# buq2/camera_calibrator

Hardware: AMD Instinct MI355X
Metric: LM residuals/sec (2*N_obs per LM iteration), single-camera intrinsics BA (higher is better)
Workload: dtype f64; 1 GPU; BASELINE.json configs[2]: single-camera intrinsics, 1000 frames x 500 pts per GPU, radial-tangential distortion, Zhang init, reference solver options (calibrator.cpp:314-321); frames_total=1000, points_per_frame=500, observations_total=500000, parallelism=frame-sharded x1, exchange=none

## Files before the change

camera_calibrator_amd/csrc/cc_intrinsics.hip:

```cpp
#include "cc_common.hpp"
#include "cc_device.hpp"
#include "cc_intrinsics_dev.hpp"
#include "cc_intrinsics_persist.hpp"


#include <algorithm>
#include <chrono>
#include <climits>
#include <cstdlib>
#include <cstring>
#include <vector>

namespace cc {

__global__ __launch_bounds__(kSweepThreads, 4) void k_intr_sweep(IntrDev P, int flags) {
  extern __shared__ __attribute__((aligned(16))) char smem_raw[];
  double* s_stage = reinterpret_cast<double*>(smem_raw);
  double* s_blk = s_stage;
  double* sm = s_stage + 4 * kStageDoublesPerWave;
  const int tid = threadIdx.x, lane = tid & 63, wave = tid >> 6;
  const int T = P.T;
  const int64_t f = (int64_t)blockIdx.x / T;
  const int tile = (int)(blockIdx.x - f * T);
  const bool in_solve = (flags & 1) != 0, restart = (flags & 2) != 0;
// ... 863 lines not shown
}

namespace cc {
int intr_create_impl(cc_intrinsics* h, const int64_t* off, const float* uv, const float* xyz);
static thread_local bool g_create_one_shot = false;
static thread_local bool g_create_no_obs = false;
static thread_local size_t g_create_extra = 0;
struct OneShotCreate {
  OneShotCreate(size_t extra, bool no_obs = false) { g_create_one_shot = true; g_create_extra = extra; g_create_no_obs = no_obs; }
  ~OneShotCreate() { g_create_one_shot = false; g_create_extra = 0; g_create_no_obs = false; }
};
static double ms_since(std::chrono::steady_clock::time_point t0) { return std::chrono::duration<double, std::milli>(std::chrono::steady_clock::now() - t0).count(); }
}

extern "C" {

void cc_intrinsics_destroy(cc_intrinsics* h);

int cc_intrinsics_create(int32_t device, int64_t F, const int64_t* off, const float* uv,
                         const float* xyz, cc_intrinsics** out) {
  using namespace cc;
  if (!out || !off || F <= 0) return fail(CC_ERR_BAD_ARGUMENT, "cc_intrinsics_create: bad arguments");
  if (off[0] != 0) return fail(CC_ERR_BAD_ARGUMENT, "frame_offsets[0] must be 0");
  for (int64_t f = 0; f < F; ++f)
    if (off[f + 1] < off[f]) return fail(CC_ERR_BAD_ARGUMENT, "frame_offsets must be non-decreasing");
  const int64_t N = off[F];
  if (F >= ((int64_t)1 << 28) || N >= ((int64_t)1 << 40))
    return fail(CC_ERR_BAD_ARGUMENT, "cc_intrinsics_create: problem too large (frames < 2^28, observations < 2^40)");
  if (N > 0 && (!uv || !xyz) && !cc::g_create_no_obs) return fail(CC_ERR_BAD_ARGUMENT, "uv/xyz are NULL");
  if (int rc = select_device(device)) return rc;
  cc_intrinsics* h = new cc_intrinsics();
  h->device = device; h->F = F; h->N = N;
  h->one_shot = cc::g_create_one_shot;
  h->no_obs_upload = cc::g_create_no_obs;
  h->extra_bytes = cc::g_create_extra;
  const int rc_init = cc::intr_create_impl(h, off, uv, xyz);
  if (rc_init != CC_OK) {
    cc_intrinsics_destroy(h);
    return rc_init;
  }
  *out = h;
  return CC_OK;
}

int cc_intrinsics_exchange_export(cc_intrinsics* h, uint8_t handle[64]) {
  using namespace cc;
  if (h && handle && h->huber_a > 0.0) return fail(CC_ERR_STATE, "cc_intrinsics_exchange_export: the handle has a Huber loss set (one device only)");
  if (h && handle && h->model != CC_MODEL_RADTAN) return fail(CC_ERR_STATE, "cc_intrinsics_exchange_export: the handle has the fisheye model set (one device only)");
  if (int rc = exchange_export_begin(h, handle, "cc_intrinsics_exchange_export")) return rc;
  h->d.x = P2pDev{};
  return mailbox_export(&h->mailbox, kVecSolve, 16, handle);
}

int cc_intrinsics_exchange_attach(cc_intrinsics* h, int32_t rank, int32_t nranks, const uint8_t* handles) {
  using namespace cc;
  if (!h || !handles || rank < 0 || nranks < 1 || rank >= nranks || nranks > kP2pMaxRanks)
    return fail(CC_ERR_BAD_ARGUMENT, "cc_intrinsics_exchange_attach: bad arguments (nranks must be 1..%d)", kP2pMaxRanks);
  if (h->huber_a > 0.0) return fail(CC_ERR_STATE, "cc_intrinsics_exchange_attach: the handle has a Huber loss set (one device only)");
  if (h->model != CC_MODEL_RADTAN) return fail(CC_ERR_STATE, "cc_intrinsics_exchange_attach: the handle has the fisheye model set (one device only)");
  if (!h->mailbox.local) return fail(CC_ERR_STATE, "cc_intrinsics_exchange_attach: call cc_intrinsics_exchange_export first");
  if (h->comm) return fail(CC_ERR_STATE, "cc_intrinsics_exchange_attach: an RCCL communicator is already attached");
  CC_HIP(hipSetDevice(h->device));
  drop_graphs(h);
  if (int rc = mailbox_attach(&h->mailbox, rank, nranks, handles, &h->d.x)) return rc;
  h->d.rank = rank;
  h->d.nranks = nranks;
  h->exchange = true;
  h->persist_x_ok = false;
  if (h->persist_ok) {
    int ndev = 1;
    if (hipGetDeviceCount(&ndev) != hipSuccess || ndev < 1) ndev = 1;
    const int co = getenv("CC_INTR_CO_RESIDENT") ? std::max(1, atoi(getenv("CC_INTR_CO_RESIDENT"))) : (nranks + ndev - 1) / ndev;
    h->persist_x_ok = (int64_t)(h->pq.G + 1) * co <= h->p_resident;
  }
  if (nranks > 1) {
    double* d_out = nullptr;
    int* d_ok = nullptr;
    CC_HIP(hipMalloc(&d_out, sizeof(double)));
    CC_HIP(hipMalloc(&d_ok, sizeof(int)));
    hipLaunchKernelGGL(k_intr_flag_exchange, dim3(1), dim3(64), 0, h->stream, h->d, h->persist_x_ok ? 1.0 : 0.0, d_out, d_ok);
    double sum = 0.0;
    int ok = 0;
    const hipError_t e1 = hipMemcpyAsync(&sum, d_out, sizeof(double), hipMemcpyDeviceToHost, h->stream);
    const hipError_t e2 = hipMemcpyAsync(&ok, d_ok, sizeof(int), hipMemcpyDeviceToHost, h->stream);
    const hipError_t e3 = hipStreamSynchronize(h->stream);
    hipFree(d_out);
    hipFree(d_ok);
    CC_HIP(e1); CC_HIP(e2); CC_HIP(e3);
    if (!ok) return fail(CC_ERR_COMM, "cc_intrinsics_exchange_attach: a peer rank did not attach within 10 s");
    h->persist_x_ok = sum == (double)nranks;
  }
  return CC_OK;
}

}

namespace cc {
int intr_create_impl(cc_intrinsics* h, const int64_t* off, const float* uv, const float* xyz) {
  const int64_t F = h->F, N = h->N;
  if (int rc = stream_get(h->device, &h->stream)) return rc;
  IntrDev& d = h->d;
  d.F = F; d.N = N; d.rank = 0; d.nranks = 1; d.mask = 0;
  {
    const int64_t per_frame = F > 0 ? (N + F - 1) / F : 0;
    int64_t T = std::min<int64_t>((per_frame + 2 * kSweepThreads - 1) / (2 * kSweepThreads), 256 / std::max<int64_t>(F, 1));
    if (const char* env = getenv("CC_SWEEP_TILES")) T = atoi(env);
    d.T = (int32_t)std::max<int64_t>(1, std::min<int64_t>(T, 8));
    d.tpad_ = 0;
    if (F * d.T >= (int64_t)INT32_MAX)
      return fail(CC_ERR_BAD_ARGUMENT, "cc_intrinsics_create: %lld frames x %d sweep tiles exceed the launch grid", (long long)F, (int)d.T);
  }
  const size_t FT = (size_t)F * d.T;
  const size_t n1 = (size_t)std::max<int64_t>(N, 1);
  size_t cursor = 0;
  auto take = [&](size_t bytes) { const size_t at = cursor; cursor += (bytes + 255) & ~(size_t)255; return at; };
  d.log_cap = 4096;
  const size_t o_intr = take(2 * 16 * sizeof(double));
  const size_t o_pose = take((size_t)2 * F * 8 * sizeof(double));
  const size_t o_stats = take(FT * kStatsCols * sizeof(double));
  const size_t o_hd0 = take(FT * 16 * sizeof(double));
  const size_t o_sp = take((size_t)F * 8 * sizeof(double));
  const size_t o_Y = take((size_t)F * kYStride * sizeof(double));
  const size_t o_partial = take((size_t)kElimMaxBlocks * kPartialCols * sizeof(double));
  const size_t o_vs = take(kVecSolve * sizeof(double));
  const size_t o_vd = take(16 * sizeof(double));
  const size_t o_ds = take(16 * sizeof(double));
  const size_t o_ss = take(16 * sizeof(double));
  const size_t o_ctl = take(sizeof(LmCtl));
  const size_t o_ctln = take(sizeof(LmCtl));
  const size_t o_sync = take(64);
  const size_t o_opts = take(sizeof(LmOpts));
  const size_t o_iintr = take(16 * sizeof(double));
  const size_t o_ipose = take((size_t)F * 8 * sizeof(double));
  int p_teams = 0;
  const bool want_persist = d.T == 1 && !(getenv("CC_INTR_PERSIST") && atoi(getenv("CC_INTR_PERSIST")) == 0);
  if (want_persist) {
    for (int t = 1; t <= kPMaxTeams && !p_teams; t *= 2) {
      int resident = 0;
      if (int rc = persist_resident_workgroups(h->device, t, &resident)) return rc;
      if ((F + t - 1) / t + 1 <= resident && (F + t - 1) / t <= kPMaxWorkers) { p_teams = t; h->p_resident = resident; }
    }
    if (const char* e = getenv("CC_INTR_PERSIST_TEAMS")) {
      const int t = atoi(e);
      int resident = 0;
      if ((t == 1 || t == 2 || t == 4) && !persist_resident_workgroups(h->device, t, &resident) && (F + t - 1) / t + 1 <= resident && (F + t - 1) / t <= kPMaxWorkers) { p_teams = t; h->p_resident = resident; }
    }
  }
  const int64_t PG = p_teams ? (F + p_teams - 1) / p_teams : 1;
  const size_t pgn = (size_t)PG;
  const size_t o_pbox0 = cursor;
  const size_t o_sbox = take(pgn * 2 * kPStatCols * sizeof(unsigned long long));
  const size_t o_pbox = take(pgn * 2 * kPartialCols * sizeof(unsigned long long));
  const size_t o_rbox = take(pgn * 2 * kPartialCols * sizeof(unsigned long long));
  const size_t o_lbox = take(((pgn + kPLeaderRows - 1) / kPLeaderRows) * 2 * kPartialCols * sizeof(unsigned long long));
  const size_t o_xbox = take(kPBcastWords * sizeof(unsigned long long));
  const size_t o_pfail = take(64);
  h->p_box_bytes = cursor - o_pbox0;
  const size_t zeroed = cursor;
  const size_t o_blocks = take((size_t)2 * FT * 256 * sizeof(double));
  const size_t o_log = take((size_t)d.log_cap * sizeof(cc_iteration));
  const size_t o_uv = take(n1 * 2 * sizeof(float));
  const size_t o_xyz = take(n1 * 3 * sizeof(float));
  const size_t o_off = take((size_t)(F + 1) * sizeof(int64_t));
  const size_t o_extra = take(h->extra_bytes);
  if (int rc = arena_get(h->device, cursor, &h->arena, &h->arena_cached)) return rc;
  char* base = static_cast<char*>(h->arena);
  h->extra = h->extra_bytes ? base + o_extra : nullptr;
  CC_HIP(hipMemsetAsync(base, 0, zeroed, h->stream));
  if (N > 0 && !h->no_obs_upload) {
    CC_HIP(hipMemcpyAsync(base + o_uv, uv, (size_t)N * 2 * sizeof(float), hipMemcpyHostToDevice, h->stream));
    CC_HIP(hipMemcpyAsync(base + o_xyz, xyz, (size_t)N * 3 * sizeof(float), hipMemcpyHostToDevice, h->stream));
  }
  CC_HIP(hipMemcpyAsync(base + o_off, off, (size_t)(F + 1) * sizeof(int64_t), hipMemcpyHostToDevice, h->stream));
  if (!h->one_shot) CC_HIP(hipStreamSynchronize(h->stream));
  d.uv = reinterpret_cast<const float*>(base + o_uv);
  d.xyz = reinterpret_cast<const float*>(base + o_xyz);
  d.off = reinterpret_cast<const int64_t*>(base + o_off);
  d.intr = reinterpret_cast<double*>(base + o_intr);
  d.pose = reinterpret_cast<double*>(base + o_pose);
  d.blocks = reinterpret_cast<double*>(base + o_blocks);
  d.stats = reinterpret_cast<double*>(base + o_stats);
  d.hd0 = reinterpret_cast<double*>(base + o_hd0);
  d.sp = reinterpret_cast<double*>(base + o_sp);
  d.Y = reinterpret_cast<double*>(base + o_Y);
  d.partial = reinterpret_cast<double*>(base + o_partial);
  d.vec_solve = reinterpret_cast<double*>(base + o_vs);
  d.vec_decide = reinterpret_cast<double*>(base + o_vd);
  d.ds = reinterpret_cast<double*>(base + o_ds);
  d.ss = reinterpret_cast<double*>(base + o_ss);
  d.ctl = reinterpret_cast<LmCtl*>(base + o_ctl);
  d.ctl_next = reinterpret_cast<LmCtl*>(base + o_ctln);
  d.arrive = reinterpret_cast<unsigned*>(base + o_sync);
  d.pub_seq = reinterpret_cast<unsigned long long*>(base + o_sync + 8);
  d.opts = reinterpret_cast<LmOpts*>(base + o_opts);
  d.log = reinterpret_cast<cc_iteration*>(base + o_log);
  h->init_intr = reinterpret_cast<double*>(base + o_iintr);
  h->init_pose = reinterpret_cast<double*>(base + o_ipose);
  d.init_intr = h->init_intr;
  d.init_pose = h->init_pose;
  static_assert(16 + sizeof(LmCtl) <= 192 && sizeof(LmCtl) <= 160 && sizeof(LmOpts) <= 160, "one cached 512-byte pinned block holds all three");
  h->pinned = pinned_block_get();
  if (!h->pinned) return fail(CC_ERR_HIP, "hipHostMalloc failed");
  h->host_pub = reinterpret_cast<volatile unsigned long long*>(h->pinned);
  h->h_ctl = reinterpret_cast<LmCtl*>(static_cast<char*>(h->pinned) + 192);
  h->h_opts = reinterpret_cast<LmOpts*>(static_cast<char*>(h->pinned) + 352);
  h->host_pub[0] = 0ull;
  h->pub_count = 0;
  {
    void* dev_view = nullptr;
    CC_HIP(hipHostGetDevicePointer(&dev_view, h->pinned, 0));
    d.host_pub = reinterpret_cast<unsigned long long*>(dev_view);
  }
  h->pq.sbox = reinterpret_cast<unsigned long long*>(base + o_sbox);
  h->pq.pbox = reinterpret_cast<unsigned long long*>(base + o_pbox);
  h->pq.rbox = reinterpret_cast<unsigned long long*>(base + o_rbox);
  h->pq.xbox = reinterpret_cast<unsigned long long*>(base + o_xbox);
  h->pq.fail = reinterpret_cast<unsigned*>(base + o_pfail);
  h->pq.lbox = reinterpret_cast<unsigned long long*>(base + o_lbox);
  h->pq.G = (int32_t)PG;
  h->pq.teams = p_teams;
  h->p_epoch = 0;
  h->persist_ok = p_teams != 0;
  h->elim_blocks = (int)std::min<int64_t>(kElimMaxBlocks, (F + 15) / 16);
  CC_HIP(hipFuncSetAttribute(reinterpret_cast<const void*>(k_intr_sweep),
                             hipFuncAttributeMaxDynamicSharedMemorySize, kSweepLdsBytes));
  CC_HIP(hipFuncSetAttribute(reinterpret_cast<const void*>(k_intr_sweep_huber),
                             hipFuncAttributeMaxDynamicSharedMemorySize, kSweepLdsBytes));
  CC_HIP(hipFuncSetAttribute(reinterpret_cast<const void*>(k_intr_sweep_fisheye),
                             hipFuncAttributeMaxDynamicSharedMemorySize, kSweepLdsBytes));
  return CC_OK;
}
}

extern "C" {

void cc_intrinsics_destroy(cc_intrinsics* h) {
  if (h) cc::last_call_status_record(h->ran_form >= 0 ? h->ran_form : cc_intrinsics_solver_form(h), h->form_reruns, h->form_note);
  if (!h) return;
  hipSetDevice(h->device);
  bool stream_ok = true;
  if (h->stream) {
    hipStreamCaptureStatus cap = hipStreamCaptureStatusNone;
    stream_ok = hipStreamSynchronize(h->stream) == hipSuccess &&
                hipStreamIsCapturing(h->stream, &cap) == hipSuccess && cap == hipStreamCaptureStatusNone;
    (void)hipGetLastError();
  }
  cc::drop_graphs(h);
  for (auto e : h->events) hipEventDestroy(e);
  if (h->comm) cc::comm_destroy(h->comm);
  cc::exchange_release(h);
  if (h->arena) cc::arena_put(h->device, h->arena, h->arena_cached);
  cc::pinned_block_put(h->pinned);
  if (stream_ok) cc::stream_put(h->device, h->stream);
  else if (h->stream) hipStreamDestroy(h->stream);
  delete h;
}

int cc_intrinsics_set_state(cc_intrinsics* h, const double* intr9, uint32_t mask, const double* q,
                            const double* t) {
  using namespace cc;
  if (!h || !intr9 || !q || !t) return fail(CC_ERR_BAD_ARGUMENT, "cc_intrinsics_set_state: NULL argument");
  CC_HIP(hipSetDevice(h->device));
  std::vector<double> pose((size_t)h->F * 8, 0.0);
  for (int64_t f = 0; f < h->F; ++f) {
    for (int i = 0; i < 4; ++i) pose[f * 8 + i] = q[f * 4 + i];
    for (int i = 0; i < 3; ++i) pose[f * 8 + 4 + i] = t[f * 3 + i];
  }
  double k[16] = {0};
  for (int i = 0; i < 9; ++i) k[i] = intr9[i];
  if (h->model == CC_MODEL_FISHEYE) { k[8] = 0.0; mask |= 1u << 8; }
  CC_HIP(hipStreamSynchronize(h->stream));
  CC_HIP(hipMemcpy(h->init_intr, k, sizeof(k), hipMemcpyHostToDevice));
  CC_HIP(hipMemcpy(h->init_pose, pose.data(), pose.size() * sizeof(double), hipMemcpyHostToDevice));
  if (h->d.mask != (mask & 0x1ffu)) drop_graphs(h);
  h->d.mask = mask & 0x1ffu;
  h->have_state = true;
  return cc_intrinsics_reset(h);
}

int cc_intrinsics_reset(cc_intrinsics* h) {
  using namespace cc;
  if (!h || !h->have_state) return fail(CC_ERR_STATE, "cc_intrinsics_reset: no state set");
  h->ctl_fresh = true;
  h->reset_pending = true;
  return CC_OK;
}

int cc_intrinsics_get_state(cc_intrinsics* h, double* intr9, double* q, double* t) {
  using namespace cc;
  if (!h) return fail(CC_ERR_BAD_ARGUMENT, "cc_intrinsics_get_state: NULL handle");
  CC_HIP(hipSetDevice(h->device));
  LmCtl c;
  if (int rc = read_ctl(h, &c)) return rc;
  const int cur = c.cur & 1;
  if (intr9) CC_HIP(hipMemcpy(intr9, h->d.intr + cur * 16, 9 * sizeof(double), hipMemcpyDeviceToHost));
  if (q || t) {
    std::vector<double> pose((size_t)h->F * 8);
    CC_HIP(hipMemcpy(pose.data(), h->d.pose + (size_t)cur * h->F * 8, pose.size() * sizeof(double), hipMemcpyDeviceToHost));
    for (int64_t f = 0; f < h->F; ++f) {
      if (q) for (int i = 0; i < 4; ++i) q[f * 4 + i] = pose[f * 8 + i];
      if (t) for (int i = 0; i < 3; ++i) t[f * 3 + i] = pose[f * 8 + 4 + i];
    }
  }
  return CC_OK;
}

int cc_intrinsics_eval(cc_intrinsics* h, double* blocks, double* cost) {
// ... 726 lines not shown
```

camera_calibrator_amd/csrc/cc_intrinsics_persist.hip:

```cpp
#include "cc_intrinsics_persist.hpp"
#include "cc_persist_dev.hpp"

namespace cc {


constexpr int persist_lds_doubles(int teams) { return teams * 4 * kStageDoublesPerWave + teams * 2 * 256 + teams * 192 + 512; }

enum { TM_Y = 0, TM_POSE = 60, TM_SP = 76, TM_STEP = 84, TM_R = 100, TM_T = 109, TM_KC = 112, TM_STEP2 = 122, TM_XN2 = 123,
       TM_QW = 124, TM_STAT = 128  };
enum { WG_INTR = 0 , WG_X = 64 , WG_DS = 66 ,
       WG_SS = 80 , WG_R0 = 96 , WG_OPT = 100 ,
       WG_TAB = 104 ,
       WG_TGI = 416 , WG_TZ = 456  };

static_assert(TM_POSE - TM_Y >= 6 * 10 && TM_SP - TM_POSE >= 2 * 8 && TM_STEP - TM_SP >= 6 && TM_R - TM_STEP >= 15 && TM_T - TM_R >= 9 && TM_KC - TM_T >= 3 &&
              TM_STEP2 - TM_KC >= 9 && TM_QW - TM_XN2 >= 1 && TM_STAT - TM_QW >= 4 && TM_STAT + 4 + 9 <= 192,
              "per-team scratch: Y (6 x 10), two poses, pose scale, step (9 + 6), R, t, intrinsics, scalars, statistics row -- inside the 192 doubles persist_lds_doubles gives a team");
static_assert(WG_X - WG_INTR >= 2 * 16 && WG_DS - WG_X >= 2 && WG_SS - WG_DS >= 9 && WG_R0 - WG_SS >= 9 && WG_OPT - WG_R0 >= 1 && WG_TAB - WG_OPT >= 4 &&
              WG_TZ - WG_TGI >= 80 / 2 && WG_TZ + 80 / 2 <= 512,
              "workgroup scratch: both intrinsics, broadcast (2 + 9), scales, options, tables of the 80-slot row -- inside the 512 doubles of persist_lds_doubles");

template <int NC, int NG, int BATCH = 8>
__device__ __forceinline__ void gather_rows(const u64* box, int G, unsigned tag, int ncols, int maxcol, double* s_part,
                                            double* out, unsigned* fail, int* s_ok, int tshift) {
  const int tid = threadIdx.x, col = tid % NC, grp = tid / NC;
  if (tid == 0) *s_ok = 1;
  __syncthreads();
  if (grp < NG && col < ncols) {
    double acc = 0.0;
    bool good = true;
    const long long t0 = wall_clock64();
    for (int r0 = grp; r0 < G && good; r0 += BATCH * NG) {
      u64 lo[BATCH], hi[BATCH];
      for (unsigned spins = 0;; ++spins) {
#pragma unroll
        for (int u = 0; u < BATCH; ++u) {
          const int r = r0 + u * NG;
          const u64* p = box + (size_t)(r < G ? r : r0) * (2 * NC) + 2 * col;
          lo[u] = ag_ld(p);
          hi[u] = ag_ld(p + 1);
        }
        bool ok = true;
#pragma unroll
        for (int u = 0; u < BATCH; ++u) ok = ok && (unsigned)(lo[u] >> 32) == tag && (unsigned)(hi[u] >> 32) == tag;
        if (ok) break;
        if ((spins & 63u) == 63u && (timed_out(t0, tshift) || ag_ld32(fail) != 0u)) { good = false; break; }
        __builtin_amdgcn_s_sleep(1);
      }
      if (!good) break;
#pragma unroll
      for (int u = 0; u < BATCH; ++u) {
        if (r0 + u * NG < G) {
          const double v = ungranule(lo[u], hi[u]);
          acc = col == maxcol ? fmax(acc, v) : acc + v;
        }
      }
    }
    s_part[grp * NC + col] = acc;
    if (!good) *s_ok = 0;
  }
  __syncthreads();
  if (tid < ncols) {
    double a = 0.0;
    if (tid == maxcol) { for (int g = 0; g < NG; ++g) a = fmax(a, s_part[g * NC + tid]); }
    else { for (int g = 0; g < NG; ++g) a += s_part[g * NC + tid]; }
    out[tid] = a;
  }
  __syncthreads();
}

template <int THREADS>
__device__ __forceinline__ void gather_stats4(const u64* box, int G, unsigned tag, double* s_part, double* out, unsigned* fail, int* s_ok, int tshift) {
  constexpr int RPT = 1024 / THREADS;
  static_assert(THREADS / 4 * RPT == kPMaxWorkers, "one statistics row per four threads: the host caps the worker grid at kPMaxWorkers");
  const int tid = threadIdx.x, col = tid & 3, lane = tid & 63, wave = tid >> 6;
  if (tid == 0) *s_ok = 1;
  __syncthreads();
  u64 lo[RPT], hi[RPT];
  bool good = true;
  const long long t0 = wall_clock64();
  for (unsigned spins = 0;; ++spins) {
    bool ok = true;
#pragma unroll
    for (int k = 0; k < RPT; ++k) {
      const int r = (tid >> 2) + k * (THREADS / 4);
      const u64* p = box + (size_t)(r < G ? r : 0) * (2 * kPStatCols) + 2 * col;
      lo[k] = ag_ld(p);
      hi[k] = ag_ld(p + 1);
    }
#pragma unroll
    for (int k = 0; k < RPT; ++k) ok = ok && (unsigned)(lo[k] >> 32) == tag && (unsigned)(hi[k] >> 32) == tag;
    if (ok) break;
    if ((spins & 63u) == 63u && (timed_out(t0, tshift) || ag_ld32(fail) != 0u)) { good = false; break; }
    __builtin_amdgcn_s_sleep(1);
  }
  double acc = 0.0;
#pragma unroll
  for (int k = 0; k < RPT; ++k)
    if ((tid >> 2) + k * (THREADS / 4) < G) acc += ungranule(lo[k], hi[k]);
  acc = wave_sum_mod<2>(acc);
  if (lane < 4) s_part[wave * 4 + lane] = acc;
  if (!good) *s_ok = 0;
  __syncthreads();
  if (tid < 4) {
    double a = 0.0;
#pragma unroll
    for (int w = 0; w < THREADS / 64; ++w) a += s_part[w * 4 + tid];
    out[tid] = a;
  }
  __syncthreads();
}

template <int THREADS>
__device__ __forceinline__ void persist_control(const IntrDev& P, const PersistDev& Q, double* lds) {
  double* s_part = lds;
  double* sv = lds + 1024;
  double* s_tot = lds + 1152;
  double* s_bc = lds + 1168;
  double* s_intr = lds + 1184;
  double* s_ss = lds + 1216;
  LmCtl* s_ctl = reinterpret_cast<LmCtl*>(lds + 1232);
  LmOpts* s_opts = reinterpret_cast<LmOpts*>(lds + 1252);
  cc_iteration* s_log = reinterpret_cast<cc_iteration*>(lds + 1264);
  int* s_int = reinterpret_cast<int*>(lds + 1296);
  const int tid = threadIdx.x, wave = tid >> 6;
  static_assert(sizeof(cc_iteration) <= 32 * 8, "log record scratch");
  if (tid < (int)(sizeof(LmCtl) / 8)) reinterpret_cast<double*>(s_ctl)[tid] = 0.0;
  if (tid >= 32 && tid < 32 + (int)(sizeof(LmOpts) / 8)) reinterpret_cast<u64*>(s_opts)[tid - 32] = reinterpret_cast<const u64*>(P.opts)[tid - 32];
  if (tid >= 64 && tid < 64 + 32) s_intr[tid - 64] = 0.0;
  __syncthreads();
  if (tid < 9) s_intr[tid] = (Q.restart ? P.init_intr : P.intr)[tid];
  if (tid == 0) s_int[1] = 0;
  __syncthreads();
  const LmOpts& o = *s_opts;
  const uint32_t mask = P.mask;

  for (int round = 0; round < Q.max_rounds; ++round) {
    const unsigned e1 = Q.epoch0 + 3u * (unsigned)round + 1u, e2 = e1 + 1u, e3 = e1 + 2u;
    const bool phase0 = round == 0;
    if (phase0) gather_rows<kPStatCols, THREADS / kPStatCols>(Q.sbox, Q.G, e1, 13, -1, s_part, s_tot, Q.fail, s_int, (phase0 ? Q.first_shift : Q.timeout_shift));
    else gather_stats4<THREADS>(Q.sbox, Q.G, e1, s_part, s_tot, Q.fail, s_int, (phase0 ? Q.first_shift : Q.timeout_shift));
    if (P.x.on) {
      const bool need = phase0 || (s_ctl->cand_pending && s_ctl->step_valid);
      if (need) {
        if (tid >= 13 && tid < 16) s_tot[tid] = 0.0;
        __syncthreads();
        const unsigned long long epoch = P.x.seq[1] + 1ull;
        p2p_post(P.x, 1, epoch, P.rank, P.nranks, s_tot, 16);
        int* s_ok2 = s_int + 4;
        const double a = p2p_collect(P.x, 1, epoch, P.rank, P.nranks, 16, s_ok2);
        if (tid < 16) s_tot[tid] = a;
        if (tid == 0) { P.x.seq[1] = epoch; if (!*s_ok2) s_int[0] = 0; }
        __syncthreads();
      }
    }
    if (tid == 0) {
      LmCtl c = *s_ctl;
      const int len0 = c.log_len, prev_cur = c.cur & 1, was_valid = c.step_valid;
      const double prev_radius = c.radius;
      const double* kc0 = s_intr + (c.cur ? 16 : 0);
      const double* kc1 = s_intr + (c.cur ? 0 : 16);
      if (!s_int[0]) {
        __hip_atomic_store(Q.fail, 1u, __ATOMIC_RELAXED, __HIP_MEMORY_SCOPE_AGENT);
        c.done = 1; c.term = CC_FAILURE_EXCHANGE;
      } else if (phase0) {
        double xn2 = s_tot[ST_XNORM2];
#pragma unroll
        for (int i = 0; i < 9; ++i) {
          const double ki = kc0[i];
          xn2 += ki * ki;
          s_ss[i] = o.jacobi_scaling ? 1.0 / (1.0 + sqrt(s_tot[4 + i])) : 1.0;
        }
        lm_init(c, o, s_tot[ST_COST], sqrt(xn2));
      } else if (c.cand_pending) {
        double step2 = s_tot[ST_STEP2], xn2 = s_tot[ST_XNORM2];
        if (c.step_valid) {
#pragma unroll
          for (int i = 0; i < 9; ++i) {
            const double kc = kc1[i], k0 = kc0[i];
            const double d = kc - k0;
            step2 += d * d;
            xn2 += kc * kc;
          }
        }
        lm_decide(c, o, s_log, s_tot[ST_COST], s_tot[ST_QMODEL], step2, xn2);
      }
      if (!c.done && round + 1 >= Q.max_rounds) { c.done = 1; c.term = CC_NO_CONVERGENCE; }
      *s_ctl = c;
      s_int[1] = c.log_len != len0;
      s_int[2] = phase0 ? (!c.done && c.radius == o.initial_radius)
                        : (was_valid && !c.done && (c.cur & 1) == (prev_cur ^ 1) && c.radius == persist_spec_radius(prev_radius, o.max_radius));
      s_bc[0] = (double)((c.done ? 1 : 0) | ((c.cur & 1) << 3));
      s_bc[1] = c.radius;
#pragma unroll
      for (int i = 0; i < 9; ++i) s_bc[2 + i] = 0.0;
    }
    __syncthreads();
    const bool hit = s_int[2] != 0;
    if (s_ctl->done || !hit) {
      if (tid < 22) ag_st(Q.xbox + tid, granule(e2, s_bc[tid >> 1], tid & 1));
      if (s_ctl->done) {
        if (tid == 0 && s_int[1] && s_ctl->log_len <= P.log_cap) P.log[s_ctl->log_len - 1] = *s_log;
        break;
      }
    }
    const unsigned erow = hit ? e2 : e3;
    gather_rows<kPartialCols, THREADS / kPartialCols, (kPLeaderRows + THREADS / kPartialCols - 1) / (THREADS / kPartialCols)>(Q.lbox, (Q.G + kPLeaderRows - 1) / kPLeaderRows, erow, kPartialCols, PC_GMAXP, s_part, sv, Q.fail, s_int, (phase0 ? Q.first_shift : Q.timeout_shift));
    if (P.x.on) {
      if (tid >= kPartialCols && tid < kVecSolve) sv[tid] = 0.0;
      __syncthreads();
      if (tid == 0) { sv[kPartialCols + P.rank] = sv[PC_GMAXP]; sv[PC_GMAXP] = 0.0; }
      __syncthreads();
      const unsigned long long epoch = P.x.seq[0] + 1ull;
      p2p_post(P.x, 0, epoch, P.rank, P.nranks, sv, kVecSolve);
      int* s_ok2 = s_int + 4;
      const double a = p2p_collect(P.x, 0, epoch, P.rank, P.nranks, kVecSolve, s_ok2);
      if (tid < kVecSolve) sv[tid] = a;
      if (tid == 0) { P.x.seq[0] = epoch; if (!*s_ok2) s_int[0] = 0; }
      __syncthreads();
      if (tid == 0) {
        double g = 0.0;
        for (int r = 0; r < P.nranks && r < 32; ++r) g = fmax(g, sv[kPartialCols + r]);
        sv[PC_GMAXP] = g;
      }
      __syncthreads();
    }
    if (wave == 0) {
      int lane = tid & 63;
      asm volatile("" : "+v"(lane));
      const int cur = s_ctl->cur & 1;
      const double radius = s_ctl->radius;
      const double gl = (lane < 9 && !((mask >> lane) & 1u)) ? fabs(sv[PC_GS + lane]) : sv[PC_GMAXP];
      const double k_l = s_intr[cur * 16 + (lane < 9 ? lane : 8)], ss_l = s_ss[lane < 9 ? lane : 8];
      bool ok = !(sv[PC_FAIL] > 0.0);
      double x[9];
      {
#pragma clang fp contract(off)
        const int i = lane < 9 ? lane : 8;
        const bool pin_i = (mask >> i) & 1u;
        const double si = s_ss[i];
        const double damp = clampd(sv[PC_HDIAG + i] * (si * si), o.min_lm_diagonal, o.max_lm_diagonal) / radius;
        double a[9];
#pragma unroll
        for (int k = 0; k < 9; ++k) {
          const int kk = k <= i ? k : i;
          const int idx = kk * 9 - kk * (kk - 1) / 2 + (i - kk);
          double v = sv[idx] * (s_ss[kk] * si);
          if (k == i) v += damp;
          const bool pin_k = (mask >> kk) & 1u;
          if (pin_i || pin_k) v = (k == i) ? 1.0 : 0.0;
          a[k] = v;
        }
        const double b = pin_i ? 0.0 : sv[PC_B + i] * si;
        ok = chol_solve_rows<9>(a, b, x) && ok;
#pragma unroll
        for (int j = 0; j < 9; ++j) ok = ok && isfinite(x[j]);
      }
      const double gmax = row16_max(gl);
      const bool go = s_int[0] && !(gmax <= o.gradient_tolerance) && !(radius < o.min_radius);
      if (lane < 9) {
        double xs = 0.0;
#pragma unroll
        for (int j = 0; j < 9; ++j) xs = lane == j ? x[j] : xs;
        const double ds = go ? -xs : 0.0;
        const double d = ((mask >> lane) & 1u) ? 0.0 : ds * ss_l;
        s_bc[2 + lane] = d;
        s_intr[(cur ^ 1) * 16 + lane] = k_l + d;
      }
      if (lane == 0) {
        s_bc[0] = (double)((go ? 0 : 1) | (go && ok ? 2 : 0) | (hit ? 4 : 0) | (cur << 3));
        s_bc[1] = radius;
        s_bc[12] = gmax;
      }
      wave_lds_fence();
      if (lane < 22) ag_st(Q.xbox + lane, granule(erow, s_bc[lane >> 1], lane & 1));
    }
    if (tid == 0) {
      const double gmax = s_bc[12];
      const bool ok = ((int)s_bc[0] & 2) != 0;
      cc_iteration* e = s_int[1] ? s_log : nullptr;
      if (e && e->accepted) e->gradient_max_norm = gmax;
      if (!s_int[0]) { __hip_atomic_store(Q.fail, 1u, __ATOMIC_RELAXED, __HIP_MEMORY_SCOPE_AGENT); s_ctl->done = 1; s_ctl->term = CC_FAILURE_EXCHANGE; }
      else if (lm_finalize(*s_ctl, o, gmax)) { s_ctl->step_valid = ok ? 1 : 0; s_ctl->cand_pending = 1; }
      if (e && s_ctl->log_len <= P.log_cap) P.log[s_ctl->log_len - 1] = *e;
    }
    __syncthreads();
    if (s_ctl->done) break;
  }
  __syncthreads();
  if (tid < 32 && ag_ld32(Q.fail) == 0u) P.intr[tid] = s_intr[tid];
  if (tid == 0) {
    LmCtl c = *s_ctl;
    if (ag_ld32(Q.fail) != 0u) { c.done = 1; c.term = CC_FAILURE_EXCHANGE; }
    if (!c.done) { c.done = 1; c.term = CC_NO_CONVERGENCE; }
    *P.ctl = c;
    *P.ctl_next = c;
    publish_to_host(P, c);
  }
}

template <int TEAMS>
__global__ __launch_bounds__(TEAMS * 256, TEAMS) void k_intr_persist(IntrDev P, PersistDev Q) {
  constexpr int THREADS = TEAMS * 256;
  extern __shared__ __attribute__((aligned(16))) char smem_raw[];
  double* s_stage = reinterpret_cast<double*>(smem_raw);
  if ((int)blockIdx.x == Q.G) { persist_control<THREADS>(P, Q, s_stage); return; }
  double* s_G = s_stage + TEAMS * 4 * kStageDoublesPerWave;
  double* s_tm = s_G + TEAMS * 2 * 256;
  double* s_wg = s_tm + TEAMS * 192;
#define CC_FRESH_TID(name) int name = tid0; asm volatile("" : "+v"(name))
  const int tid0 = threadIdx.x, wave = __builtin_amdgcn_readfirstlane(tid0 >> 6), team = wave >> 2, twave = wave & 3;
  const int sbase = (team & 3) * 64;
  const int64_t f = (int64_t)blockIdx.x * TEAMS + team;
  const bool has_frame = f < P.F;
  double* sm = s_tm + team * 192;
  double* tstage = s_stage + team * 4 * kStageDoublesPerWave;
  double* s_blk = tstage;
  double* Zs = tstage + 1024;
  double* red = tstage + 1100;
  unsigned char* pj = reinterpret_cast<unsigned char*>(s_wg + WG_TAB);
  unsigned char* pk = pj + 48;
  const uint32_t mask = P.mask;

  {
  const int tid = tid0, ttid = tid0 & 255;
  if (has_frame && ttid < 8) {
    const double v = ttid < 7 ? (Q.restart ? P.init_pose : P.pose)[(size_t)f * 8 + ttid] : 0.0;
    sm[TM_POSE + ttid] = v;
    sm[TM_POSE + 8 + ttid] = v;
  }
  if (ttid >= 64 && ttid < 64 + 60) sm[TM_Y + ttid - 64] = 0.0;
  if (tid < 32) s_wg[WG_INTR + tid] = 0.0;
  if (tid == 32) {
    const LmOpts* o = P.opts;
    s_wg[WG_OPT] = o->jacobi_scaling ? 1.0 : 0.0;
    s_wg[WG_OPT + 1] = o->min_lm_diagonal;
    s_wg[WG_OPT + 2] = o->max_lm_diagonal;
    s_wg[WG_OPT + 3] = o->max_radius;
    s_wg[WG_R0] = o->initial_radius;
  }
  if (tid == 33) {
    int oo = 0;
    for (int j = 0; j < 9; ++j)
      for (int k = j; k < 9; ++k) { pj[oo] = (unsigned char)j; pk[oo] = (unsigned char)k; ++oo; }
  }
  if (tid >= 64 && tid < 64 + 16) s_wg[WG_X + tid - 64] = 0.0;
  if (tid >= 80 && tid < 80 + 16) s_wg[WG_SS + tid - 80] = 1.0;
  __syncthreads();
  if (tid < 9) s_wg[WG_INTR + tid] = (Q.restart ? P.init_intr : P.intr)[tid];
  if (tid >= 128 && tid < 128 + kPartialCols) {
    const int o = tid - 128;
    int gi = 0, z = 0;
    if (o < 45) {
      const int j = pj[o], k = pk[o];
      gi = j * 16 + k; z = j | (k << 8) | (1 << 16);
    } else if (o < 54) {
      const int j = o - 45;
      gi = j * 16 + 15; z = j | (9 << 8) | (1 << 16);
    } else if (o < 63) {
      const int j = o - 54;
// ... 146 lines not shown
        sm[TM_STAT + ST_QMODEL] = (sm[TM_QW] + sm[TM_QW + 1]) + (sm[TM_QW + 2] + sm[TM_QW + 3]);
        sm[TM_STAT + ST_STEP2] = sm[TM_STEP2];
        sm[TM_STAT + ST_XNORM2] = sm[TM_XN2];
      }
      if (phase0 && ttid < 9 * 17 && ttid % 17 == 0) sm[TM_STAT + 4 + ttid / 17] = g;
      __syncthreads();
    }
    {
      CC_FRESH_TID(tid);
      const int ncols = phase0 ? 13 : 4;
      const int stid = tid - 128;
      if (stid >= 0 && stid < 2 * ncols) {
        const int c = stid >> 1;
        double a = 0.0;
        if (do_sweep) {
#pragma unroll
          for (int k = 0; k < TEAMS; ++k)
            if ((int64_t)blockIdx.x * TEAMS + k < P.F) a += s_tm[k * 192 + TM_STAT + c];
        }
        ag_st(Q.sbox + (size_t)blockIdx.x * (2 * kPStatCols) + stid, granule(e1, a, stid & 1));
      }
    }
    auto eliminate_and_post = [&](const int cur_e, const double radius_e, const bool first, u64* box, const unsigned tag) {
    CC_FRESH_TID(tid_e);
    if (has_frame && (tid_e & 255) >= sbase && (tid_e & 255) < sbase + 16) {
      const int l = (tid_e & 255) - sbase;
      const double* Gl = s_G + (team * 2 + cur_e) * 256;
      const double* ss = s_wg + WG_SS;
      const bool jac = s_wg[WG_OPT] != 0.0;
      const double mn = s_wg[WG_OPT + 1], mx = s_wg[WG_OPT + 2];
      const double inv_radius = 1.0 / radius_e;
      double s[6], L[21];
#pragma unroll
      for (int i = 0; i < 6; ++i)
#pragma unroll
        for (int j = 0; j <= i; ++j) L[tri(i, j)] = Gl[(9 + i) * 16 + 9 + j];
      if (first) {
#pragma unroll
        for (int i = 0; i < 6; ++i) s[i] = jac ? 1.0 / (1.0 + sqrt(L[tri(i, i)])) : 1.0;
        if (l < 6) {
          double sl = 0.0;
#pragma unroll
          for (int i = 0; i < 6; ++i) sl = l == i ? s[i] : sl;
          sm[TM_SP + l] = sl;
        }
      } else {
#pragma unroll
        for (int i = 0; i < 6; ++i) s[i] = sm[TM_SP + i];
      }
#pragma unroll
      for (int i = 0; i < 6; ++i)
#pragma unroll
        for (int j = 0; j <= i; ++j) L[tri(i, j)] = s[i] * L[tri(i, j)] * s[j];
#pragma unroll
      for (int i = 0; i < 6; ++i) L[tri(i, i)] += clampd(L[tri(i, i)], mn, mx) * inv_radius;
      bool ok = true;
      double Li[6];
#pragma unroll
      for (int j = 0; j < 6; ++j) {
        double d = L[tri(j, j)];
#pragma unroll
        for (int k = 0; k < j; ++k) d -= L[tri(j, k)] * L[tri(j, k)];
        ok = ok && (d > 0.0) && isfinite(d);
        const double inv = rsqrt_pos(d);
        L[tri(j, j)] = d * inv;
        Li[j] = inv;
#pragma unroll
        for (int i = j + 1; i < 6; ++i) {
          double a = L[tri(i, j)];
#pragma unroll
          for (int k = 0; k < j; ++k) a -= L[tri(i, k)] * L[tri(j, k)];
          L[tri(i, j)] = a * inv;
        }
      }
#pragma unroll
      for (int i = 0; i < 21; ++i) L[i] = rfl(L[i]);
#pragma unroll
      for (int i = 0; i < 6; ++i) { Li[i] = rfl(Li[i]); s[i] = rfl(s[i]); }
      if (l < 10) {
        const double sc = l < 9 ? ss[l] : 1.0;
        const int col = l < 9 ? l : 15;
        double w[6], z[6], y[6];
#pragma unroll
        for (int i = 0; i < 6; ++i) w[i] = Gl[(9 + i) * 16 + col];
#pragma unroll
        for (int i = 0; i < 6; ++i) {
          double a = s[i] * w[i] * sc;
#pragma unroll
          for (int k = 0; k < i; ++k) a -= L[tri(i, k)] * z[k];
          z[i] = a * Li[i];
        }
#pragma unroll
        for (int i = 5; i >= 0; --i) {
          double a = z[i];
#pragma unroll
          for (int k = i + 1; k < 6; ++k) a -= L[tri(k, i)] * y[k];
          y[i] = a * Li[i];
        }
#pragma unroll
        for (int i = 0; i < 6; ++i) {
          Zs[i * 10 + l] = z[i];
          sm[TM_Y + i * 10 + l] = y[i];
        }
      }
      if (l == 0) red[PC_FAIL] = ok ? 0.0 : 1.0;
    }
    if (has_frame && (tid_e & 255) >= sbase && (tid_e & 255) < sbase + 64) {
      const int l64 = (tid_e & 255) - sbase;
      const double* Gl = s_G + (team * 2 + cur_e) * 256;
      wave_lds_fence();
      const int* tgi = reinterpret_cast<const int*>(s_wg + WG_TGI);
      const int* tz = reinterpret_cast<const int*>(s_wg + WG_TZ);
      double accv[2];
      int zz_[2];
#pragma unroll
      for (int r = 0; r < 2; ++r) {
        const int o = l64 + 64 * r, oc = o < kPartialCols ? o : 0;
        zz_[r] = tz[oc];
        accv[r] = Gl[tgi[oc]];
      }
#pragma unroll
      for (int r = 0; r < 2; ++r) {
        const int zj = zz_[r] & 255, zk = (zz_[r] >> 8) & 255;
        double zz = 0.0;
#pragma unroll
        for (int i = 0; i < 6; ++i) zz += Zs[i * 10 + zj] * Zs[i * 10 + zk];
        const int o = l64 + 64 * r;
        const bool used = o < 63 || (o >= PC_GS && o < PC_GS + 9);
        if (o < kPartialCols && o != PC_FAIL && o != PC_GMAXP) red[o] = used ? accv[r] - ((zz_[r] >> 16) ? zz : 0.0) : 0.0;
      }
    }
    if (has_frame && (tid_e & 255) == (((team & 3) + 1) & 3) * 64) {
      const double* Gg = s_G + (team * 2 + cur_e) * 256;
      double q4[4], g6[6];
#pragma unroll
      for (int i = 0; i < 4; ++i) q4[i] = sm[TM_POSE + cur_e * 8 + i];
#pragma unroll
      for (int i = 0; i < 6; ++i) g6[i] = Gg[(9 + i) * 16 + 15];
      red[PC_GMAXP] = pose_grad_proj_max_tab(q4, g6);
    }
    __syncthreads();
    {
      CC_FRESH_TID(tid);
      if (tid < 2 * kPartialCols) {
        const int c = tid >> 1;
        double a = 0.0;
#pragma unroll
        for (int k = 0; k < TEAMS; ++k) {
          if ((int64_t)blockIdx.x * TEAMS + k < P.F) {
            const double v = s_stage[k * 4 * kStageDoublesPerWave + 1100 + c];
            a = c == PC_GMAXP ? fmax(a, v) : a + v;
          }
        }
        ag_st(box + (size_t)blockIdx.x * (2 * kPartialCols) + tid, granule(tag, a, tid & 1));
      }
    }
    if ((blockIdx.x % kPLeaderRows) == 0) {
      int* s_lok = reinterpret_cast<int*>(s_wg + 250);
      const int g0 = (int)blockIdx.x, n = Q.G - g0 < kPLeaderRows ? Q.G - g0 : kPLeaderRows;
      double* lout = s_wg + 128;
      gather_rows<kPartialCols, THREADS / kPartialCols, (kPLeaderRows + THREADS / kPartialCols - 1) / (THREADS / kPartialCols)>(box + (size_t)g0 * (2 * kPartialCols), n, tag, kPartialCols, PC_GMAXP, s_stage + 2048, lout,
                                                        Q.fail, s_lok, (phase0 ? Q.first_shift : Q.timeout_shift));
      CC_FRESH_TID(tid);
      if (!*s_lok && tid == 0) __hip_atomic_store(Q.fail, 1u, __ATOMIC_RELAXED, __HIP_MEMORY_SCOPE_AGENT);
      if (*s_lok && tid < 2 * kPartialCols) ag_st(Q.lbox + (size_t)(g0 / kPLeaderRows) * (2 * kPartialCols) + tid, granule(tag, lout[tid >> 1], tid & 1));
    }
    };
    auto wait_bcast = [&](const unsigned tag) {
      CC_FRESH_TID(tid);
      if (wave == 0 && !bcast_wait(Q.xbox, tag, 11, s_wg + WG_X, Q.fail, tid & 63, (phase0 ? Q.first_shift : Q.timeout_shift))) s_wg[WG_X] = 17.0;
      __syncthreads();
    };

    const bool spec = do_sweep;
    const double radius_spec = phase0 ? s_wg[WG_R0] : persist_spec_radius(radius, s_wg[WG_OPT + 3]);
    if (spec) eliminate_and_post(dst, radius_spec, phase0, Q.pbox, e2);
    wait_bcast(e2);
    int fl = (int)s_wg[WG_X];
    if (fl & 16) failed = true;
    if (fl & 1) { cur = (fl >> 3) & 1; break; }
    if (fl & 4) {
      cur = dst;
      radius = radius_spec;
    } else {
      cur = (fl >> 3) & 1;
      radius = s_wg[WG_X + 1];
      eliminate_and_post(cur, radius, false, Q.rbox, e3);
      wait_bcast(e3);
      fl = (int)s_wg[WG_X];
      if (fl & 16) failed = true;
      if (fl & 1) { cur = (fl >> 3) & 1; break; }
    }
    step_valid = (fl & 2) != 0;
  }
  if (!failed && ag_ld32(Q.fail) == 0u && has_frame && (tid0 & 255) < 7) P.pose[((size_t)cur * P.F + f) * 8 + (tid0 & 255)] = sm[TM_POSE + cur * 8 + (tid0 & 255)];
  asm volatile("" ::"v"(nm.x), "v"(nX0), "v"(nX1), "v"(nX2));
}

template <int TEAMS>
static int resident_of(int device, int* out) {
  const int lds = persist_lds_doubles(TEAMS) * 8;
  CC_HIP(hipFuncSetAttribute(reinterpret_cast<const void*>(k_intr_persist<TEAMS>), hipFuncAttributeMaxDynamicSharedMemorySize, lds));
  int per_cu = 0, cus = 0;
  CC_HIP(hipOccupancyMaxActiveBlocksPerMultiprocessor(&per_cu, k_intr_persist<TEAMS>, TEAMS * 256, lds));
  CC_HIP(hipDeviceGetAttribute(&cus, hipDeviceAttributeMultiprocessorCount, device));
  *out = per_cu >= 1 ? cus : 0;
  return 0;
}

int persist_resident_workgroups(int device, int teams, int* out) {
  return teams == 1 ? resident_of<1>(device, out) : teams == 2 ? resident_of<2>(device, out) : resident_of<4>(device, out);
}

void persist_launch(const IntrDev& P, const PersistDev& Q, bool drop_control, hipStream_t stream) {
  const dim3 grid((unsigned)Q.G + (drop_control ? 0u : 1u));
  if (Q.teams == 1) hipLaunchKernelGGL(k_intr_persist<1>, grid, dim3(256), persist_lds_doubles(1) * 8, stream, P, Q);
  else if (Q.teams == 2) hipLaunchKernelGGL(k_intr_persist<2>, grid, dim3(512), persist_lds_doubles(2) * 8, stream, P, Q);
  else hipLaunchKernelGGL(k_intr_persist<4>, grid, dim3(1024), persist_lds_doubles(4) * 8, stream, P, Q);
}

}
```

camera_calibrator_amd/csrc/cc_intrinsics_persist.hpp:

```cpp
#pragma once
#include "cc_intrinsics_dev.hpp"

namespace cc {

constexpr int kPMaxTeams = 4;
constexpr int kPStatCols = 16;
constexpr int kPBcastWords = 64;
constexpr int kPMaxWorkers = 256;
constexpr int kPLeaderRows = 16;

struct PersistDev {
  unsigned long long* sbox;
  unsigned long long* pbox;
  unsigned long long* rbox;
  unsigned long long* lbox;
  unsigned long long* xbox;
  unsigned* fail;
  int32_t G;
  int32_t teams;
  uint32_t epoch0;
  int32_t max_rounds;
  int32_t restart;
  int32_t timeout_shift;
  int32_t first_shift;
};

int persist_resident_workgroups(int device, int teams, int* out);
void persist_launch(const IntrDev& P, const PersistDev& Q, bool drop_control, hipStream_t stream);

}
```

Baseline: 31.96 billion residuals/s.

## Replace leader-row reduction with per-column owner workgroups and column-major partial box

Switches the persistent kernel's cross-workgroup reduction of partial columns from a two-level scheme (a leader every 16 rows gathers rows, then the control block gathers the leader rows) to one where each of the first kPartialCols workgroups owns a column. Each owner uses a single wave to spin on that column's entries across all workers, stored column-major, and publishes one final total. The control block then reads only one row of totals. This shortens the dependency chain and the polling volume on the controller's critical path, at the cost of adding spin-wait work on one wave of several worker blocks and relying on the grouped summation order matching the old one.

```diff
diff --git a/camera_calibrator_amd/csrc/cc_intrinsics.hip b/camera_calibrator_amd/csrc/cc_intrinsics.hip
--- a/camera_calibrator_amd/csrc/cc_intrinsics.hip
+++ b/camera_calibrator_amd/csrc/cc_intrinsics.hip
@@ -1039,7 +1039,7 @@
   const size_t o_sbox = take(pgn * 2 * kPStatCols * sizeof(unsigned long long));
   const size_t o_pbox = take(pgn * 2 * kPartialCols * sizeof(unsigned long long));
   const size_t o_rbox = take(pgn * 2 * kPartialCols * sizeof(unsigned long long));
-  const size_t o_lbox = take(((pgn + kPLeaderRows - 1) / kPLeaderRows) * 2 * kPartialCols * sizeof(unsigned long long));
+  const size_t o_lbox = take((size_t)2 * kPartialCols * sizeof(unsigned long long));
   const size_t o_xbox = take(kPBcastWords * sizeof(unsigned long long));
   const size_t o_pfail = take(64);
   h->p_box_bytes = cursor - o_pbox0;
diff --git a/camera_calibrator_amd/csrc/cc_intrinsics_persist.hip b/camera_calibrator_amd/csrc/cc_intrinsics_persist.hip
--- a/camera_calibrator_amd/csrc/cc_intrinsics_persist.hip
+++ b/camera_calibrator_amd/csrc/cc_intrinsics_persist.hip
@@ -1,5 +1,6 @@
 #include "cc_intrinsics_persist.hpp"
 #include "cc_persist_dev.hpp"
+#include "cc_persist_sum.hpp"
 
 namespace cc {
 
@@ -107,6 +108,91 @@
 #pragma unroll
     for (int w = 0; w < THREADS / 64; ++w) a += s_part[w * 4 + tid];
     out[tid] = a;
+  }
+  __syncthreads();
+}
+
+__device__ __forceinline__ size_t persist_box_word(int c, int g, int G) {
+  return kPBoxColumnMajor ? ((size_t)c * (size_t)G + (size_t)g) * 2 : ((size_t)g * kPartialCols + (size_t)c) * 2;
+}
+
+template <int NG>
+__device__ __forceinline__ void own_columns(const u64* box, u64* obox, int G, int w, unsigned tag, double* vals, unsigned* fail, int tid0, int tshift) {
+  constexpr int kPer = (kPMaxWorkers + 63) / 64;
+  int lane = tid0 & 63;
+  asm volatile("" : "+v"(lane));
+  asm volatile("" : "+s"(G));
+  const int nc = (kPartialCols - 1 - w) / G + 1, items = nc * G, nL = persist_sum_groups(G);
+  const u64* p[kPer];
+#pragma unroll
+  for (int u = 0; u < kPer; ++u) {
+    const int i = lane + 64 * u, ic = i < items ? i : 0, k = ic / G;
+    p[u] = box + persist_box_word(w + k * G, ic - k * G, G);
+  }
+  int gv[2], gn[2], gm[2];
+#pragma unroll
+  for (int u = 0; u < 2; ++u) {
+    const int t = lane + 64 * u, tc = t < nc * nL ? t : 0, k = tc / nL, j = tc - k * nL;
+    gv[u] = k * G + j * kPSumRows;
+    gn[u] = persist_sum_group_rows(G, j);
+    gm[u] = w + k * G == PC_GMAXP;
+  }
+  asm volatile("" : "+v"(gv[0]), "+v"(gv[1]), "+v"(gn[0]), "+v"(gn[1]), "+v"(gm[0]), "+v"(gm[1]));
+  u64 lo[kPer], hi[kPer];
+  bool good = true;
+  const long long t0 = wall_clock64();
+  for (unsigned spins = 0;; ++spins) {
+#pragma unroll
+    for (int u = 0; u < kPer; ++u) {
+      lo[u] = ag_ld(p[u]);
+      hi[u] = ag_ld(p[u] + 1);
+    }
+    bool ok = true;
+#pragma unroll
+    for (int u = 0; u < kPer; ++u) ok = ok && (unsigned)(lo[u] >> 32) == tag && (unsigned)(hi[u] >> 32) == tag;
+    if (ok) break;
+    if ((spins & 63u) == 63u && (timed_out(t0, tshift) || ag_ld32(fail) != 0u)) { good = false; break; }
+    __builtin_amdgcn_s_sleep(1);
+  }
+  if (__any(!good)) {
+    if (lane == 0) __hip_atomic_store(fail, 1u, __ATOMIC_RELAXED, __HIP_MEMORY_SCOPE_AGENT);
+    return;
+  }
+#pragma unroll
+  for (int u = 0; u < kPer; ++u)
+    if (lane + 64 * u < items) vals[lane + 64 * u] = ungranule(lo[u], hi[u]);
+  wave_lds_fence();
+  double* Ls = vals + kPMaxWorkers + kPSumRows;
+#pragma unroll
+  for (int u = 0; u < 2; ++u)
+    if (lane + 64 * u < nc * nL) Ls[lane + 64 * u] = persist_sum_group<NG>(vals + gv[u], gn[u], gm[u] != 0);
+  wave_lds_fence();
+  for (int k = lane; k < nc; k += 64) {
+    const int c = w + k * G;
+    const double total = persist_sum_group<NG>(Ls + k * nL, nL, c == PC_GMAXP);
+    ag_st(obox + 2 * c, granule(tag, total, 0));
+    ag_st(obox + 2 * c + 1, granule(tag, total, 1));
+  }
+}
+
+__device__ __forceinline__ void gather_totals(const u64* box, unsigned tag, double* out, unsigned* fail, int* s_ok, int tshift) {
+  const int tid = threadIdx.x;
+  if (tid == 0) *s_ok = 1;
+  __syncthreads();
+  if (tid < kPartialCols) {
+    const u64* p = box + 2 * tid;
+    u64 lo, hi;
+    bool good = true;
+    const long long t0 = wall_clock64();
+    for (unsigned spins = 0;; ++spins) {
+      lo = ag_ld(p);
+      hi = ag_ld(p + 1);
+      if ((unsigned)(lo >> 32) == tag && (unsigned)(hi >> 32) == tag) break;
+      if ((spins & 63u) == 63u && (timed_out(t0, tshift) || ag_ld32(fail) != 0u)) { good = false; break; }
+      __builtin_amdgcn_s_sleep(1);
+    }
+    out[tid] = ungranule(lo, hi);
+    if (!good) *s_ok = 0;
   }
   __syncthreads();
 }
@@ -205,7 +291,7 @@
       }
     }
     const unsigned erow = hit ? e2 : e3;
-    gather_rows<kPartialCols, THREADS / kPartialCols, (kPLeaderRows + THREADS / kPartialCols - 1) / (THREADS / kPartialCols)>(Q.lbox, (Q.G + kPLeaderRows - 1) / kPLeaderRows, erow, kPartialCols, PC_GMAXP, s_part, sv, Q.fail, s_int, (phase0 ? Q.first_shift : Q.timeout_shift));
+    gather_totals(Q.lbox, erow, sv, Q.fail, s_int, (phase0 ? Q.first_shift : Q.timeout_shift));
     if (P.x.on) {
       if (tid >= kPartialCols && tid < kVecSolve) sv[tid] = 0.0;
       __syncthreads();
@@ -658,19 +744,11 @@
             a = c == PC_GMAXP ? fmax(a, v) : a + v;
           }
         }
-        ag_st(box + (size_t)blockIdx.x * (2 * kPartialCols) + tid, granule(tag, a, tid & 1));
-      }
-    }
-    if ((blockIdx.x % kPLeaderRows) == 0) {
-      int* s_lok = reinterpret_cast<int*>(s_wg + 250);
-      const int g0 = (int)blockIdx.x, n = Q.G - g0 < kPLeaderRows ? Q.G - g0 : kPLeaderRows;
-      double* lout = s_wg + 128;
-      gather_rows<kPartialCols, THREADS / kPartialCols, (kPLeaderRows + THREADS / kPartialCols - 1) / (THREADS / kPartialCols)>(box + (size_t)g0 * (2 * kPartialCols), n, tag, kPartialCols, PC_GMAXP, s_stage + 2048, lout,
-                                                        Q.fail, s_lok, (phase0 ? Q.first_shift : Q.timeout_shift));
-      CC_FRESH_TID(tid);
-      if (!*s_lok && tid == 0) __hip_atomic_store(Q.fail, 1u, __ATOMIC_RELAXED, __HIP_MEMORY_SCOPE_AGENT);
-      if (*s_lok && tid < 2 * kPartialCols) ag_st(Q.lbox + (size_t)(g0 / kPLeaderRows) * (2 * kPartialCols) + tid, granule(tag, lout[tid >> 1], tid & 1));
-    }
+        ag_st(box + persist_box_word(tid >> 1, (int)blockIdx.x, Q.G) + (tid & 1), granule(tag, a, tid & 1));
+      }
+    }
+    if (wave == 3 && (int)blockIdx.x < kPartialCols)
+      own_columns<THREADS / kPartialCols>(box, Q.lbox, Q.G, (int)blockIdx.x, tag, s_stage + 2048, Q.fail, tid0, (phase0 ? Q.first_shift : Q.timeout_shift));
     };
     auto wait_bcast = [&](const unsigned tag) {
       CC_FRESH_TID(tid);
diff --git a/camera_calibrator_amd/csrc/cc_intrinsics_persist.hpp b/camera_calibrator_amd/csrc/cc_intrinsics_persist.hpp
--- a/camera_calibrator_amd/csrc/cc_intrinsics_persist.hpp
+++ b/camera_calibrator_amd/csrc/cc_intrinsics_persist.hpp
@@ -7,7 +7,7 @@
 constexpr int kPStatCols = 16;
 constexpr int kPBcastWords = 64;
 constexpr int kPMaxWorkers = 256;
-constexpr int kPLeaderRows = 16;
+constexpr bool kPBoxColumnMajor = true;
 
 struct PersistDev {
   unsigned long long* sbox;
diff --git a/camera_calibrator_amd/csrc/cc_persist_sum.hpp b/camera_calibrator_amd/csrc/cc_persist_sum.hpp
--- /dev/null
+++ b/camera_calibrator_amd/csrc/cc_persist_sum.hpp
@@ -0,0 +1,44 @@
+#pragma once
+#include <math.h>
+
+#ifdef __HIPCC__
+#define CC_PSUM_FN __host__ __device__ __forceinline__
+#else
+#define CC_PSUM_FN inline
+#endif
+
+namespace cc {
+
+constexpr int kPSumRows = 16;
+
+CC_PSUM_FN int persist_sum_groups(int G) { return (G + kPSumRows - 1) / kPSumRows; }
+CC_PSUM_FN int persist_sum_group_rows(int G, int j) { return G - j * kPSumRows < kPSumRows ? G - j * kPSumRows : kPSumRows; }
+
+template <int NG, bool IS_MAX>
+CC_PSUM_FN double persist_sum_group_of(const double* v, int n) {
+  constexpr int kPer = (kPSumRows + NG - 1) / NG;
+  double x[kPSumRows];
+#pragma unroll
+  for (int r = 0; r < kPSumRows; ++r) x[r] = v[r];
+#pragma unroll
+  for (int r = 0; r < kPSumRows; ++r) x[r] = r < n ? x[r] : 0.0;
+  double total = 0.0;
+#pragma unroll
+  for (int g = 0; g < NG; ++g) {
+    double a = 0.0;
+#pragma unroll
+    for (int u = 0; u < kPer; ++u) {
+      const int r = g + u * NG;
+      if (r < kPSumRows) a = IS_MAX ? fmax(a, x[r]) : a + x[r];
+    }
+    total = IS_MAX ? fmax(total, a) : total + a;
+  }
+  return total;
+}
+
+template <int NG>
+CC_PSUM_FN double persist_sum_group(const double* v, int n, bool is_max) {
+  return is_max ? persist_sum_group_of<NG, true>(v, n) : persist_sum_group_of<NG, false>(v, n);
+}
+
+}
```

Result: faster. 32.94 billion residuals/s, median of 6 (+3.0%).
